# hucancode/hello-raytracing

Hardware: AMD Instinct MI355X
Metric: Mrays/sec at 1920x1080x1024spp x 50-bounce (RTIOW cover scene) (higher is better)
Workload: dtype f32

## Files before the change

hello-raytracing_amd/csrc/rt_kernels.hip:

```cpp
#include "rt_device.hpp"
#include "rt_tile_lists.hpp"

#include <algorithm>
#include <type_traits>

using namespace hrt_dev;

namespace {

struct Ray {
    f3 o, d;
};

#ifdef HRT_STAMPS
__device__ __forceinline__ unsigned long long hrt_stamp() {
    unsigned long long t;
    __builtin_amdgcn_sched_barrier(0);
    asm volatile("s_memtime %0\n\ts_waitcnt lgkmcnt(0)" : "=s"(t)::"memory");
    __builtin_amdgcn_sched_barrier(0);
    return t;
}
__device__ __forceinline__ unsigned long long hrt_realtime() {
    unsigned long long t;
    __builtin_amdgcn_sched_barrier(0);
// ... 237 lines not shown
    const float a4 = 4.0f * a, a2 = 2.0f * a;
    Q.sp = 0;
    const bool finite_o = __builtin_isfinite(r.o.x) && __builtin_isfinite(r.o.y) && __builtin_isfinite(r.o.z);
    if (!(a2 > 0x1p-100f && a2 < 0x1p100f) || !finite_o) {
        Q.full_scan = 1u;
        return false;
    }
    Q.full_scan = 0u;
    const uint32_t nleaf = P.bvh_nleaf;
    float bt = best;
    int bc = -1;
    KPtr K = nullptr;
    if constexpr (LLDS) K = kargs();
    const uint32_t nlarge = LLDS ? K->bq_nlarge : KA ? kargs()->nlarge : P.nlarge;
    if constexpr (LLDS) {
        static_assert(KA && FAST, "k_trace_split's begin");
        for (uint32_t k = 0, n = min(nlarge, LLARGE_CAP); k < n; k++) {
            const float4 g = lgeo[k];
            const bool cand = sphere_candidate(g, r, a4);
            const float t = candidate_t(g, r, a4, a2, cand);
            if (cand && t > 0.0f && t < bt) { bt = t; bc = (int)(nleaf + k); }
        }
    } else
    for (uint32_t k = 0; k < nlarge; k++) {
        const int i = P.large_slots[k];
        float t;
        if constexpr (FAST) {
            const float4 g = P.sph_geo[i];
            const bool cand = sphere_candidate(g, r, a4);
            t = candidate_t(g, r, a4, a2, cand);
            t = cand ? t : -1.0f;
        } else {
            t = exact_t_geo<false>(P.sph_geo[i], r, a4, a2);
        }
        if (beats(t, i, bt, bc >= 0 ? bvh_slot_of(P, bc) : -1)) { bt = t; bc = (int)(nleaf + k); }
    }
    if constexpr (COUNT) tally.spheres += nlarge;
    Q.bt = bt;
    Q.bc = bc;
    if constexpr (LLDS) {
        bvh_slab_k<SO>(r, Q, K->bq_rc, K->bq_rr_h, K->bq_k1, K->bq_k2, K->bq_k3, K->bq_k4);
    } else {
        bvh_slab<SO>(P, r, Q);
    }
    Q.node = P.bvh_root;
    return true;
}

template <bool SO, typename RC>
__device__ __forceinline__ void bvh_slab_k(const Ray& r, BvhQuery& Q, RC rc, float rr, float k1, float k2, float k3, float k4) {
    const float a = dot(r.d, r.d);
    const f3 op = mk(r.o.x - rc[0], r.o.y - rc[1], r.o.z - rc[2]);
    const float dl = __builtin_amdgcn_sqrtf(dot(op, op));
    const float D = dl * 1.001f + rr;
    const float delta = k1 + fmin_ieee(k2 * (D * D), k3 * D) + k4 * D +
                        4.0001e-23f * __builtin_amdgcn_rsqf(a);
    const float pad = 2.02f * delta;
    Q.S.inv = mk(robust_inv(r.d.x), robust_inv(r.d.y), robust_inv(r.d.z));
    if constexpr (SO) {
        const f3 ps = mk(__builtin_copysignf(pad, Q.S.inv.x), __builtin_copysignf(pad, Q.S.inv.y),
                         __builtin_copysignf(pad, Q.S.inv.z));
        Q.S.lo = mk(-op.x - ps.x, -op.y - ps.y, -op.z - ps.z);
        Q.S.hi = mk(-op.x + ps.x, -op.y + ps.y, -op.z + ps.z);
    } else {
        Q.S.lo = mk(-op.x - pad, -op.y - pad, -op.z - pad);
        Q.S.hi = mk(-op.x + pad, -op.y + pad, -op.z + pad);
    }
    Q.S.lo = Q.S.lo * Q.S.inv;
    Q.S.hi = Q.S.hi * Q.S.inv;
}

typedef _Float16 hrt_h2 __attribute__((ext_vector_type(2)));
__device__ __forceinline__ float h16_lo(uint32_t u) { return (float)__builtin_bit_cast(hrt_h2, u).x; }
__device__ __forceinline__ float h16_hi(uint32_t u) { return (float)__builtin_bit_cast(hrt_h2, u).y; }
__device__ __forceinline__ void load_hnode(const uint4* __restrict__ hn, uint32_t node, float4& n0, float4& n1,
                                           float4& n2, float4& n3) {
    const uint4 c0 = hn[2 * node], c1 = hn[2 * node + 1];
    n0 = float4{h16_lo(c0.x), h16_lo(c0.y), h16_lo(c0.z), __uint_as_float(c0.w)};
    n1 = float4{h16_hi(c0.x), h16_hi(c0.y), h16_hi(c0.z), 0.0f};
    n2 = float4{h16_lo(c1.x), h16_lo(c1.y), h16_lo(c1.z), __uint_as_float(c1.w)};
    n3 = float4{h16_hi(c1.x), h16_hi(c1.y), h16_hi(c1.z), 0.0f};
}

__device__ __forceinline__ bool box_hit_so(uint32_t px, uint32_t py, uint32_t pz, uint32_t shx, uint32_t shy, uint32_t shz,
                                           const Slab& S, float bt, float& tenter) {
    const uint32_t x = __builtin_amdgcn_alignbit(px, px, shx), y = __builtin_amdgcn_alignbit(py, py, shy),
                   z = __builtin_amdgcn_alignbit(pz, pz, shz);
    const float tnx = __builtin_fmaf(h16_lo(x), S.inv.x, S.lo.x), tfx = __builtin_fmaf(h16_hi(x), S.inv.x, S.hi.x);
    const float tny = __builtin_fmaf(h16_lo(y), S.inv.y, S.lo.y), tfy = __builtin_fmaf(h16_hi(y), S.inv.y, S.hi.y);
    const float tnz = __builtin_fmaf(h16_lo(z), S.inv.z, S.lo.z), tfz = __builtin_fmaf(h16_hi(z), S.inv.z, S.hi.z);
    const float tmin = fmax_ieee(fmax_ieee(tnx, tny), fmax_ieee(tnz, 0.0f));
    const float tmax = fmin_ieee(fmin_ieee(tfx, tfy), tfz);
    tenter = tmin;
    return tmin <= tmax && tmin <= bt;
}

template <bool FAST>
__device__ __forceinline__ void leaf_sphere_test(const KParams& P, const Ray& r, float a4, float a2, uint32_t i, float& bt,
                                                 int& bc) {
    float4 g;
    if constexpr (FAST) {
        typedef float f4v __attribute__((ext_vector_type(4)));
        const __amdgpu_buffer_rsrc_t rs =
            __builtin_amdgcn_make_buffer_rsrc((void*)P.bvh_sph, (short)0, (int)(P.bvh_nleaf * 16u), 0x00020000);
        const f4v v = __builtin_amdgcn_raw_buffer_load_b128(rs, (int)(i * 16u), 0, 0);
        g = float4{v.x, v.y, v.z, v.w};
    } else {
        g = P.bvh_sph[i];
    }
    const float t = exact_t_geo<FAST>(g, r, a4, a2);
    if (t > 0.0f && t <= bt) {
        int slot;
        if constexpr (FAST) {
            const __amdgpu_buffer_rsrc_t rsl =
                __builtin_amdgcn_make_buffer_rsrc((void*)P.bvh_slot, (short)0, (int)(P.bvh_nleaf * 4u), 0x00020000);
            slot = (int)__builtin_amdgcn_raw_buffer_load_b32(rsl, (int)(i * 4u), 0, 0);
        } else {
            slot = P.bvh_slot[i];
        }
        if (t < bt || (bc >= 0 && slot < bvh_slot_of(P, bc))) { bt = t; bc = (int)i; }
    }
}

template <bool SUSPEND, bool SELECT, uint32_t LS, bool COUNT = true, bool HOLD = false, bool PAIR = false,
          typename SW = uint32_t>
__device__ __forceinline__ bool bvh_walk_noovf(const KParams& P, const Ray& r, BvhQuery& Q, SW* stack, Tally& tally,
                                               uint32_t below, const uint4* __restrict__ hn, uint32_t hold = 0u) {
    constexpr bool S16 = sizeof(SW) == 2;
    const Slab S = Q.S;
    const uint32_t shx = (__float_as_uint(S.inv.x) >> 27) & 16u, shy = (__float_as_uint(S.inv.y) >> 27) & 16u,
                   shz = (__float_as_uint(S.inv.z) >> 27) & 16u;
    const float a = dot(r.d, r.d);
    const float a4 = 4.0f * a, a2 = 2.0f * a;
    uint32_t node = Q.node;
    int sp = Q.sp;
    float bt = Q.bt;
    int bc = Q.bc;
    uint32_t finished = 0u;
#ifdef HRT_STAMPS
    tally.lentry++;
    if (first_active_lane()) tally.wentry++;
#endif
    while (true) {
#ifdef HRT_STAMPS
        tally.lwalk++;
        if (first_active_lane()) tally.wwalk++;
#endif
        uint32_t lim = 0u;
        if constexpr (HOLD) lim = min(hold, (uint32_t)__popcll(__ballot(1)));
        constexpr uint32_t BVH_MISS = 0xFFFFFFFFu;
        if (!(node & BVH_LEAF_BIT)) {
            bool any;
            do {
#ifdef HRT_STAMPS
                {
                    constexpr uint32_t DIAG_LOW = 24u;
                    const bool low = (uint32_t)__popcll(__ballot(1)) < DIAG_LOW;
                    tally.lbox++;
                    tally.lbox_low += low ? 1u : 0u;
                    if (first_active_lane()) {
                        tally.wbox++;
                        tally.wbox_low += low ? 1u : 0u;
                    }
                }
#endif
                float tl, tr;
                const uint4 c0 = hn[2 * node], c1 = hn[2 * node + 1];
                const bool hl = box_hit_so(c0.x, c0.y, c0.z, shx, shy, shz, S, bt, tl);
                const bool hr = box_hit_so(c1.x, c1.y, c1.z, shx, shy, shz, S, bt, tr);
                if constexpr (COUNT) tally.boxes += 2;
                const bool lfirst = hl && (!hr || tl <= tr);
                const uint32_t near = lfirst ? c0.w : c1.w, far = lfirst ? c1.w : c0.w;
                const bool both = hl && hr;
                any = hl || hr;
                stack[sp * LS] = (SW)far;
                sp += both ? 1 : 0;
                node = any ? near : (HOLD ? BVH_MISS : node);
                if constexpr (HOLD) {
                    const unsigned long long wants = __builtin_amdgcn_ballot_w64(!(node & BVH_LEAF_BIT));
                    if (!__builtin_amdgcn_inverse_ballot_w64((uint32_t)__popcll(wants) < lim ? 0ull : wants)) break;
                } else {
                    if (!(any && !(node & BVH_LEAF_BIT))) break;
                }
            } while (true);
        }
        if (HOLD ? (int32_t)node < -1 : (node & BVH_LEAF_BIT) != 0u) {
#ifdef HRT_STAMPS
            {
                constexpr uint32_t DIAG_LOW = 24u;
                const bool low = (uint32_t)__popcll(__ballot(1)) < DIAG_LOW;
                tally.lleaf++;
                tally.lleaf_low += low ? 1u : 0u;
                if (first_active_lane()) {
                    tally.wleaf++;
                    tally.wleaf_low += low ? 1u : 0u;
                }
            }
#endif
            const uint32_t first = (node >> 4) & (S16 ? 0x7FFu : 0x07FFFFFFu), cnt = node & 15u;
            if constexpr (SELECT) {
                typedef float f4v __attribute__((ext_vector_type(4)));
                const __amdgpu_buffer_rsrc_t rs =
                    __builtin_amdgcn_make_buffer_rsrc((void*)P.bvh_sph, (short)0, (int)(P.bvh_nleaf * 16u), 0x00020000);
                auto leaf_geo = [&](uint32_t o) -> float4 {
                    const f4v v = __builtin_amdgcn_raw_buffer_load_b128(rs, (int)o, 0, 0);
                    return float4{v.x, v.y, v.z, v.w};
                };
                uint32_t cand = 0u;
                if constexpr (PAIR) {
                    static_assert(BVH_MAX_LEAF <= 4u, "two pairs cover a leaf");
                    const uint32_t o = first * 16u;
                    HRT_TALLY(lpass1, wpass1);
                    const f4v v0 = __builtin_amdgcn_raw_buffer_load_b128(rs, (int)o, 0, 0);
                    const f4v v1 = __builtin_amdgcn_raw_buffer_load_b128(rs, (int)o, 16, 0);
                    if (sphere_candidate(float4{v0.x, v0.y, v0.z, v0.w}, r, a4)) cand |= 1u;
                    if (sphere_candidate(float4{v1.x, v1.y, v1.z, v1.w}, r, a4)) cand |= 2u;
                    if (cnt > 2u) {
                        HRT_TALLY(lpass1, wpass1);
                        const f4v v2 = __builtin_amdgcn_raw_buffer_load_b128(rs, (int)o, 32, 0);
                        const f4v v3 = __builtin_amdgcn_raw_buffer_load_b128(rs, (int)o, 48, 0);
                        if (sphere_candidate(float4{v2.x, v2.y, v2.z, v2.w}, r, a4)) cand |= 4u;
                        if (sphere_candidate(float4{v3.x, v3.y, v3.z, v3.w}, r, a4)) cand |= 8u;
                    }
                    cand &= ~(~0u << cnt);
                } else {
                    for (uint32_t o = first * 16u, oe = (first + cnt) * 16u, bit = 1u; o != oe; o += 16u, bit <<= 1) {
                        HRT_TALLY(lpass1, wpass1);
                        if (sphere_candidate(leaf_geo(o), r, a4)) cand |= bit;
                    }
                }
#ifdef HRT_STAMPS
                if (cand != 0u) HRT_TALLY(lrun, wrun);
#endif
                while (cand != 0u) {
                    HRT_TALLY(lroot, wroot);
                    const uint32_t o = (first + (uint32_t)__builtin_ctz(cand)) * 16u;
                    cand &= cand - 1u;
                    const float t = candidate_t(leaf_geo(o), r, a4, a2);
                    if (t > 0.0f && t <= bt) {
                        const __amdgpu_buffer_rsrc_t rsl = __builtin_amdgcn_make_buffer_rsrc(
                            (void*)P.bvh_slot, (short)0, (int)(P.bvh_nleaf * 4u), 0x00020000);
                        const int slot = (int)__builtin_amdgcn_raw_buffer_load_b32(rsl, (int)(o >> 2), 0, 0);
                        if (t < bt || (bc >= 0 && slot < bvh_slot_of(P, bc))) { bt = t; bc = (int)(o >> 4); }
                    }
                }
            } else {
                for (uint32_t o = first * 16u, oe = (first + cnt) * 16u; o != oe; o += 16u)
                    leaf_sphere_test<false>(P, r, a4, a2, o >> 4, bt, bc);
            }
            if constexpr (COUNT) tally.spheres += cnt;
        }
        if constexpr (HOLD) {
            const bool held = !(node & BVH_LEAF_BIT);
            const bool fin = !held && sp == 0;
            const int spn = max(sp - 1, 0);
// ... 2093 lines not shown
            } else {
                uint32_t* const rw = rows + 9u * (threadIdx.x >> 6);
                if ((lane & 7u) == 0u) rw[lane >> 3] = (x * K->cam.H + y) * time;
                if (lane == 0u) rw[8] = K->cam.H * time;
            }
            __builtin_amdgcn_fence(__ATOMIC_RELEASE, "wavefront");
            __builtin_amdgcn_wave_barrier();
            __builtin_amdgcn_fence(__ATOMIC_ACQUIRE, "wavefront");
        }
        const uint32_t avail = 64u - B.blk_next;
        const uint32_t rank = (uint32_t)__popcll(m & below);
        const uint32_t src = (B.blk_next + rank) & 63u;
        const float* const e = blk + BW * ((threadIdx.x & ~63u) + src);
        const float ox = e[0], oy = e[1], oz = e[2], dx = e[3], dy = e[4], dz = e[5];
        bool took = false;
        const uint32_t okb = (okw[2u * (threadIdx.x >> 6) + (src >> 5)] >> (src & 31u)) & 1u;
        if (need && rank < avail) {
            need = false;
            if (okb) {
                ray.o = mk(ox, oy, oz);
                ray.d = mk(dx, dy, dz);
                if constexpr (SEED) {
                    s = __float_as_uint(e[6]);
                } else {
                    const uint32_t* const rw = rows + 9u * (threadIdx.x >> 6);
                    uint32_t st = rw[src >> 3] + (src & 7u) * rw[8];
#pragma unroll
                    for (int k = 0; k < 5; k++) st = pcg_next(st);
                    s = st;
                }
                fl = sample_ref<RING>(J, B.job_f0, B.blk_f);
                pix = B.job_tile * 64u + src;
                sky_t = ray.d.y * 0.5f + 0.5f;
                att = mk(1.0f, 1.0f, 1.0f);
                bounce = 0;
                have = true;
                qs = 0;
                took = true;
            }
        }
        job_dealt<RING>(J, (uint32_t)__popcll(__ballot(took)));
        B.blk_next += min((uint32_t)__popcll(m), avail);
        if (B.blk_next == 64u && B.blk_f + 1u >= B.job_nf) job_close(J, lane);
        m = __ballot(need);
    }
}

#ifdef HRT_PHASES
#define HRT_PHASE_DECL                                                                       \
    unsigned long long ph[5] = {0, 0, 0, 0, 0}, pl[4] = {0, 0, 0, 0}, pr[4] = {0, 0, 0, 0}; \
    const unsigned long long ph_start = hrt_stamp();                                         \
    unsigned long long ph_t = ph_start
#define HRT_PHASE(k)                                                                         \
    do {                                                                                     \
        const unsigned long long t_ = hrt_stamp();                                          \
        ph[k] += t_ - ph_t;                                                                  \
        ph_t = t_;                                                                           \
    } while (0)
#define HRT_LANES(k, pred)                                                                   \
    do {                                                                                     \
        const uint32_t c_ = (uint32_t)__popcll(__ballot(pred));                              \
        if (c_) { pl[k] += c_; pr[k]++; }                                                    \
    } while (0)
#define HRT_PHASE_FLUSH                                                                      \
    if (lane == 0) {                                                                         \
        for (int k = 0; k < 4; k++) atomicAdd(P.counter + 8 + k, ph[k]);                     \
        atomicAdd(P.counter + 12, hrt_stamp() - ph_start);                                   \
        for (int k = 0; k < 3; k++) atomicAdd(P.counter + 5 + k, pl[k]);                     \
        atomicAdd(P.counter + 13, pr[0]);                                                    \
        atomicAdd(P.counter + 14, pr[2]);                                                    \
    }
#else
#define HRT_PHASE_DECL do { } while (0)
#define HRT_PHASE(k) do { } while (0)
#define HRT_LANES(k, pred) do { } while (0)
#define HRT_PHASE_FLUSH
#endif

constexpr bool split_stack16(bool lnodes, bool packet) { return lnodes && !packet; }
constexpr int split_waves(bool lnodes, bool steal, bool count, bool packet, bool ring) {
    if (packet) return steal ? 6 : 7;
    return split_stack16(lnodes, packet) && !steal && !count && !ring ? 8 : 7;
}
template <bool LNODES, bool STEAL, bool COUNT, bool PACKET, bool RING>
__device__ __forceinline__ void trace_split(const KParams& P) {
    static_assert(!PACKET || LNODES, "the packet walk reads the LDS nodes and keeps its stack in one VGPR (depth <= 8)");
    constexpr int MODE = MODE_SPHERE;
    constexpr int FM = PACKET ? FOLD_DYN : (int)RING;
    static_assert(!(PACKET && RING) && !(STEAL && RING), "no such instantiation: launch_trace_split");
    constexpr int SPLIT_STACK = LNODES ? (int)LNODE_DEPTH : 14;
    constexpr bool SHADE_BY_CODE = !PACKET;
    constexpr bool SEAMS = !PACKET && !STEAL && !RING;
    constexpr uint32_t QS_IDLE = 0xFFFFFFFFu, QS_PASS = 0xFFFFFFFEu;
    constexpr bool BLOCKRES = SEAMS && !COUNT && LNODES;
    constexpr bool WAVEQ = PACKET || BLOCKRES;
    constexpr uint32_t QS_FULL = 5u;
    const uint32_t lane = threadIdx.x & 63u;
    constexpr bool STACK16 = split_stack16(LNODES, PACKET);
    static_assert(!STACK16 || (LNODE_CAP <= 0x8000u && (LNODE_CAP + 1u) * BVH_MAX_LEAF <= 2048u),
                  "a 16-bit stack entry holds a node index or first << 4 | count in 15 bits");
    using StackWord = std::conditional_t<STACK16, int16_t, uint32_t>;
    __shared__ StackWord bvh_stack[SPLIT_STACK * 256];
    __shared__ uint4 lnodes[LNODES ? 2 * LNODE_CAP : 1];
    constexpr bool LLDS = LNODES && !PACKET;
    __shared__ float4 lgeo[LLDS ? LLARGE_CAP : 1];
    if constexpr (LNODES) {
        const uint32_t nn = 2u * min(P.bvh_nnodes, LNODE_CAP);
        for (uint32_t i = threadIdx.x; i < nn; i += 256u) {
            uint4 c = P.bvh_hnodes[i];
            if constexpr (STACK16) c.w = (uint32_t)(int32_t)(int16_t)(c.w | (c.w >> 16));
            lnodes[i] = c;
        }
        if constexpr (LLDS) {
            if (threadIdx.x < min(P.nlarge, LLARGE_CAP)) {
                lgeo[threadIdx.x] = P.sph_geo[P.large_slots[threadIdx.x]];
            }
        }
        __syncthreads();
    }
    __shared__ float4 blk[2 * 256];
    __shared__ float blk_sky[BLOCKRES ? 256 : 1];
    constexpr uint32_t EW_RES = 0x80000000u;
    Tally tally;
    uint32_t queries = 0;
    const uint32_t suspend_below = P.suspend_below & 0xFFu, hold = P.suspend_below >> 8;

    bool drained = false;
    Ray ray;
    f3 att = mk(1.0f, 1.0f, 1.0f);
    float sky_t = 0.0f;
    uint32_t s = 0, bounce = 0, pix = 0, fl = 0;
    bool have = false;
    uint32_t qs = SEAMS ? QS_IDLE : 0u;
    const auto has = [&]() { return (int)qs >= 0; };
    BvhQuery Q;
    uint32_t job_tile = 0, job_f0 = 0, job_nf = 0, blk_f = 0, blk_next = 64;
    uint32_t blk_cnt = 64;
    uint32_t nres = 0;
    uint32_t nfull = 0;
    const auto blk_n = [&]() { return BLOCKRES ? blk_cnt : 64u; };
    __shared__ uint32_t wjobs[4 * WJ_WORDS];
    const WaveJobs Jp = PACKET ? wave_jobs(wjobs) : WaveJobs{nullptr};
    StackWord* const stack_p = PACKET ? bvh_stack + threadIdx.x : nullptr;
    if (FM != 1 && P.fold_prev != nullptr) fold_prev_tiles(P, lane);
    const WaveJobs J = PACKET ? Jp : wave_jobs(wjobs);
    StackWord* const stack = PACKET ? stack_p : bvh_stack + threadIdx.x;
    const unsigned long long below = (1ull << lane) - 1ull;
    HRT_PHASE_DECL;
#ifdef HRT_STAMPS
    WaveRecord wrec;
    wrec.begin();
    uint32_t nblocks = 0;
#endif
    while (true) {
        if constexpr (SEAMS) qs = (uint32_t)max((int)qs, (int)QS_IDLE);
        bool need = (SEAMS ? qs == QS_IDLE : !have) && !drained;
        unsigned long long m = __ballot(need);
        while (m != 0ull) {
            if (blk_next == blk_n()) {
                if constexpr (STEAL) {
                    if ((uint32_t)__popcll(m) < CLAIM_FREE && J.get(WJ_PRIV_N) == 0u && __ballot(have) != 0ull &&
                        queue_drained(J, lane))
                        break;
                    if (!steal_block(J, lane, job_tile, job_f0)) {
                        drained = steal_drained(J);
                        break;
                    }
                    blk_f = 0;
                    job_nf = 1;
                } else {
                    if (J.dealing()) {
                        blk_f++;
                    } else {
                        if ((J.get(WJ_FLAGS) & WJ_TAILPH) && (uint32_t)__popcll(m) < CLAIM_FREE &&
                            __ballot(SEAMS ? has() : have) != 0ull)
                            break;
                        if (!job_acquire<FM, true>(J, lane, drained, job_tile, job_f0, job_nf)) break;
                        blk_f = 0;
                    }
                }
                blk_next = 0;
#ifdef HRT_STAMPS
                nblocks++;
#endif
                const uint32_t x = (job_tile % P.tiles_w) * 8u + (lane & 7u);
                const uint32_t kr = (job_tile / P.tiles_w) * 8u + (lane >> 3);
                const uint32_t pok = (x < P.W && kr < P.nrows) ? 1u : 0u;
                Ray pr = {mk(0.0f, 0.0f, 0.0f), mk(0.0f, 0.0f, 0.0f)};
                uint32_t ps = 0;
                uint32_t ew = pok;
                if (pok) {
                    const KPtr K = kargs();
                    uint32_t y;
                    if constexpr (SEAMS) {
                        const uint32_t rb = K->row_block, rs = K->row_stride;
                        if (__builtin_expect(rb == rs, 1)) y = K->row0 + kr;
                        else y = global_row(K->row0, rb, rs, kr);
                    } else {
                        y = global_row(K->row0, K->row_block, K->row_stride, kr);
                    }
                    pr = primary_ray<MODE>(&K->cam, x, y, K->time0 + (job_f0 + blk_f) * K->dtime, ps);
                }
                bool resolved = false;
                if constexpr (BLOCKRES) {
                    typedef const __attribute__((address_space(4))) uint32_t* CU32;
                    typedef float f4v __attribute__((ext_vector_type(4)));
                    typedef const __attribute__((address_space(4))) f4v* CF4;
                    blk_cnt = 64u;
                    const KPtr TK = kargs();
                    const CU32 tl = (CU32)TK->tile_lists + uniform(job_tile) * TILE_LIST_WORDS;
                    const uint32_t ln = TK->tile_lists != nullptr ? tl[0] : TILE_LIST_WALK;
                    const float a = dot(pr.d, pr.d);
                    const float a4 = 4.0f * a, a2 = 2.0f * a;
                    const bool cov = (a2 > 0x1p-100f && a2 < 0x1p100f) && __builtin_isfinite(pr.o.x) &&
                                     __builtin_isfinite(pr.o.y) && __builtin_isfinite(pr.o.z);
                    if (ln != TILE_LIST_WALK && __ballot(pok != 0u && !cov) == 0ull) {
                        resolved = true;
                        nres++;
                        blk[2 * threadIdx.x] = float4{ray.o.x, ray.o.y, ray.o.z, ray.d.x};
                        blk[2 * threadIdx.x + 1] = float4{ray.d.y, ray.d.z, __uint_as_float(s), __uint_as_float(pix)};
                        blk_sky[threadIdx.x] = sky_t;
                        const bool live = pok != 0u;
                        float bt = FLT_MAX_REF;
                        int bc = -1;
// ... 120 lines not shown
                            blk[2 * threadIdx.x + 1].w = __uint_as_float(rw);
                        }
                    }
                }
                __builtin_amdgcn_fence(__ATOMIC_RELEASE, "wavefront");
                __builtin_amdgcn_wave_barrier();
                __builtin_amdgcn_fence(__ATOMIC_ACQUIRE, "wavefront");
            }
            const uint32_t avail = blk_n() - blk_next;
            const uint32_t rank = WAVEQ ? __builtin_amdgcn_mbcnt_hi((uint32_t)(m >> 32), __builtin_amdgcn_mbcnt_lo((uint32_t)m, 0u))
                                         : (uint32_t)__popcll(m & below);
            const int src = (int)((blk_next + rank) & 63u);
            const float4 b0 = blk[2 * ((threadIdx.x & ~63u) + (uint32_t)src)];
            const float4 b1 = blk[2 * ((threadIdx.x & ~63u) + (uint32_t)src) + 1];
            const float ox = b0.x, oy = b0.y, oz = b0.z, dx = b0.w, dy = b1.x, dz = b1.y;
            const uint32_t ss = __float_as_uint(b1.z), ok = __float_as_uint(b1.w);
            bool took = false;
            if ((SEAMS ? qs == QS_IDLE : need) && rank < avail) {
                need = false;
                if constexpr (SEAMS) qs = QS_PASS;
                if (ok & 1u) {
                    ray.o = mk(ox, oy, oz);
                    ray.d = mk(dx, dy, dz);
                    s = ss;
                    if constexpr (SEAMS) {
                        pix = (job_f0 + blk_f) * kargs()->sample_npix + job_tile * 64u +
                              (BLOCKRES && (ok & EW_RES) ? (ok >> 1) & 63u : (uint32_t)src);
                    } else {
                        fl = sample_ref<FM>(J, job_f0, blk_f);
                        pix = job_tile * 64u + (uint32_t)src;
                    }
                    sky_t = ray.d.y * 0.5f + 0.5f;
                    att = mk(1.0f, 1.0f, 1.0f);
                    bounce = 0;
                    if constexpr (BLOCKRES) {
                        if (ok & EW_RES) {
                            const SphereAux* const w = P.code_aux + ((ok & ~EW_RES) >> 7);
                            sky_t = blk_sky[(threadIdx.x & ~63u) + (uint32_t)src];
                            att = att * mk(w->ar * 0.7f, w->ag * 0.7f, w->ab * 0.7f);
                            bounce = 1;
                        }
                    }
                    if constexpr (!SEAMS) have = true;
                    qs = 0;
                    if constexpr (PACKET) {
                        if (ok & 2u) {
                            qs = 4u;
                            Q.bc = (ok & 4u) ? (int)(ok >> 3) : -1;
                        }
                    }
                    took = true;
                }
            }
            job_dealt<FM>(J, (uint32_t)__popcll(__ballot(took)));
            blk_next += min((uint32_t)__popcll(m), avail);
            if (blk_next == blk_n() && blk_f + 1u >= job_nf) job_close(J, lane);
            m = __ballot(SEAMS ? qs == QS_IDLE : need);
        }
#ifdef HRT_STAMPS
        wrec.drain(drained);
#endif
        if (__ballot(SEAMS ? has() : have) == 0ull) {
            if (drained && J.idle()) break;
            if (!drained && idle_spin(J, lane)) break;
        }
        bool fin = false;
#ifdef HRT_STAMPS
        if (lane == 0) tally.rounds++;
#endif
        HRT_PHASE(0);
        HRT_LANES(0, (SEAMS ? has() : have) && qs == 0u);
        if (SEAMS ? qs == 0u : have && qs == 0u) {
            if (bounce < P.bounces) {
                qs = bvh_begin<true, true, true, COUNT, LLDS>(P, ray, FLT_MAX_REF, Q, tally, lgeo) ? 1u : BLOCKRES ? QS_FULL : 2u;
            } else {
                qs = 3u;
            }
        }
        HRT_PHASE(1);
        HRT_LANES(1, (SEAMS ? has() : have) && qs == 1u);
        if (SEAMS ? qs == 1u : have && qs == 1u) {
            if constexpr (LNODES) {
                constexpr bool PAIR = !PACKET && !STEAL;
                if (bvh_walk_noovf<true, true, 256, COUNT, !PACKET, PAIR>(P, ray, Q, stack, tally, suspend_below, lnodes, hold))
                    qs = 2u;
            } else {
                if (bvh_walk_ovf<true, SPLIT_STACK, true, 256, true, COUNT>(P, ray, Q, stack, tally, suspend_below, P.bvh_hnodes))
                    qs = 2u;
            }
        }
        HRT_PHASE(2);
        HRT_LANES(2, (SEAMS ? has() : have) && qs >= 2u);
        if constexpr (PACKET) queries += (uint32_t)__popcll(__ballot(have && (qs == 2u || qs == 4u)));
        if constexpr (BLOCKRES) {
            const uint32_t nf = (uint32_t)__popcll(__ballot(qs == QS_FULL));
            queries += (uint32_t)__popcll(__ballot(qs == 2u)) + nf;
            nfull += nf;
        }
        if (SEAMS ? (int)qs >= 2 : have && qs >= 2u) {
#ifdef HRT_STAMPS
            tally.lshade++;
            if (first_active_lane()) tally.wshade++;
#endif
            bool done = true;
            if (qs == 2u || (PACKET && qs == 4u) || (BLOCKRES && qs == QS_FULL)) {
                float best = FLT_MAX_REF;
                int bi;
                f3 p;
                if (PACKET && qs == 4u) {
                    bi = Q.bc;
                    p = ray.o;
                } else if constexpr (SHADE_BY_CODE) {
                    bi = Q.bc;
                    if (BLOCKRES ? qs == QS_FULL : Q.full_scan != 0u) {
                        if constexpr (BLOCKRES) {
                            bi = scan_spheres_p<false>(kargs(), ray, best);
                        } else {
                            bi = bvh_end<true>(P, ray, Q, best, tally);
                        }
                        bi = bi >= 0 ? bi + (int)(P.bvh_nleaf + kargs()->nlarge) : bi;
                    } else {
                        best = Q.bt;
                    }
                    p = point_on_ray(ray.o, ray.d, best);
                } else {
                    bi = bvh_end<true>(P, ray, Q, best, tally);
                    p = point_on_ray(ray.o, ray.d, best);
                }
                if constexpr (!WAVEQ) queries++;
                if (bi >= 0) {
                    Hit h;
                    if constexpr (SEAMS) {
                        const __amdgpu_buffer_rsrc_t rsa =
                            __builtin_amdgcn_make_buffer_rsrc((void*)P.code_aux, (short)0, (int)P.code_aux_bytes, 0x00020000);
                        const int aoff = sphere_record_rs(rsa, p, ray.d, bi, best, h);
                        scatter_dc<MODE, true>(s, ray, h, [&]() {
                            const u32x4 m = __builtin_amdgcn_raw_buffer_load_b128(rsa, aoff, 32, 0);
                            return DielRegs{__uint_as_float(m.y), __uint_as_float(m.z), __uint_as_float(m.w)};
                        });
                    } else {
                        const SphereAux* __restrict__ tab = SHADE_BY_CODE ? P.code_aux : nullptr;
                        sphere_record_p<true>(P, p, ray.d, bi, best, h, tab);
                        scatter<MODE, true>(P, s, ray, h, tab);
                    }
                    att = att * mk(h.ar * 0.7f, h.ag * 0.7f, h.ab * 0.7f);
                    bounce++;
                    done = bounce >= P.bounces;
                }
            }
            if (done) {
                const float u = 1.0f - sky_t;
                const f3 sky = mk(0.54f * u + 0.54f * sky_t, 0.86f * u + 0.7f * sky_t, 0.92f * u + 0.98f * sky_t);
                const f3 c = att * sky;
                if constexpr (SEAMS) {
                    const KPtr RK = kargs();
                    float* const o = RK->samples + (unsigned long long)pix * 3u;
#if defined(HRT_STAMPS) && defined(HRT_DIAG_NOSTORE)
                    if (c.x == -12345.0f)
#endif
                    {
                        o[0] = c.x;
                        o[1] = c.y;
                        o[2] = c.z;
                    }
                    if (uint32_t* const tc = RK->tile_cost)
                        __hip_atomic_fetch_add(tc + pix % RK->sample_npix, bounce + 1u, __ATOMIC_RELAXED, __HIP_MEMORY_SCOPE_AGENT);
                } else {
                    ring_store<FM>(J, pix, fl, c, bounce + 1u);
                }
                if constexpr (!SEAMS) have = false;
                fin = true;
            }
            qs = SEAMS && done ? QS_IDLE : 0u;
        }
        job_account<FM, 1>(J, fin, fl, lane);
        HRT_PHASE(3);
    }
#ifdef HRT_STAMPS
    wrec.finish(P, lane, nblocks);
#endif
    HRT_PHASE_FLUSH
#if defined(HRT_STAMPS) && !defined(HRT_PHASES)
    {
#ifdef HRT_LEAFSTAT
        unsigned long long v[10] = {tally.lbox, tally.wbox, tally.lleaf, tally.wleaf, tally.lpass1, tally.wpass1,
                                    tally.lrun, tally.wrun, tally.lroot, tally.wroot};
#else
        unsigned long long v[10] = {tally.lbox, tally.wbox, tally.lleaf, tally.wleaf, tally.rounds, tally.lshade,
                                    tally.wshade, tally.lwalk, tally.wwalk, tally.lentry};
#endif
#pragma unroll
        for (int c = 0; c < 10; c++) {
#pragma unroll
            for (int off = 32; off > 0; off >>= 1) v[c] += __shfl_xor(v[c], off);
        }
        if (lane == 0)
            for (int c = 0; c < 10; c++) atomicAdd(P.counter + 5 + c, v[c]);
    }
#endif
#ifdef HRT_RINGSTAT
    if (lane == 0)
        for (uint32_t c = 0; c < 4u; c++) atomicAdd(P.counter + 5 + c, (unsigned long long)J.get(WJ_STAT + c));
#endif
    if constexpr (BLOCKRES) {
        if (lane == 0) {
            unsigned long long sums[6] = {queries, 0ull, (unsigned long long)nfull * kargs()->nslots, 0ull, 0ull, nres};
            flush_counts(sums);
        }
        return;
    }
    unsigned long long sums[5] = {(!WAVEQ || lane == 0u) ? queries : 0u, tally.boxes, tally.spheres, tally.nodes, tally.tris};
#pragma unroll
    for (int c = 0; c < 5; c++) {
#pragma unroll
        for (int off = 32; off > 0; off >>= 1) sums[c] += __shfl_xor(sums[c], off);
    }
    if (lane == 0) flush_counts(sums);
}
template <bool LNODES, bool STEAL, bool COUNT, bool PACKET>
__global__ __launch_bounds__(256) __attribute__((amdgpu_waves_per_eu(split_waves(LNODES, STEAL, COUNT, PACKET, false)))) void
k_trace_split(const KParams P) {
    trace_split<LNODES, STEAL, COUNT, PACKET, false>(P);
}
template <bool LNODES, bool COUNT>
__global__ __launch_bounds__(256) __attribute__((amdgpu_waves_per_eu(split_waves(LNODES, false, COUNT, false, true)))) void
k_ring_split(const KParams P) {
    trace_split<LNODES, false, COUNT, false, true>(P);
}

constexpr uint32_t heap_wg(int hl) { return hl == 3 ? 768u : 256u; }
constexpr uint32_t heap_list_words(int hl, int scan) { return hl == 0 ? TRI_BATCH : (hl == 3 && scan != SCAN_BVH) ? 7u : 8u; }
constexpr uint32_t heap_top_n(int hl, int scan) { return hl == 0 ? 0u : hl == 1 ? 256u : 1024u; }

template <int MODE, int SCAN, int HL, bool STEAL, bool RING>
__device__ __forceinline__ void trace_split_tris(const KParams& P) {
    static_assert(MODE != MODE_SPHERE, "k_trace_split covers the sphere program");
    constexpr uint32_t WGT = heap_wg(HL), HT = heap_top_n(HL, SCAN);
    const uint32_t lane = threadIdx.x & 63u;
    constexpr uint32_t LIST_WORDS = heap_list_words(HL, SCAN);
    constexpr int SPHERE_STACK = (int)LIST_WORDS;
    static_assert(SCAN != SCAN_BVH || HL == 0 || LIST_WORDS == 8, "the culling walk's stack needs 8 entries");
    __shared__ uint32_t lane_words[LIST_WORDS * WGT];
    uint32_t* const cand = lane_words + threadIdx.x;
    uint32_t* const sstack = lane_words + threadIdx.x;
    __shared__ float heap_top[HL > 0 ? 9 * HT : 1];
    if constexpr (HL > 0) {
        const uint32_t nf = 9u * min(P.n, HT);
        for (uint32_t t = threadIdx.x; t < nf; t += WGT) heap_top[t] = P.nodes_so[t];
        __syncthreads();
    }
    uint16_t* defer_list = nullptr;
    if constexpr (SCAN == SCAN_DEFER) {
        static_assert(HL <= 1, "the deferred scan's lists assume 256-lane workgroups");
        __shared__ uint16_t defer_cand[(CAND_CAP + 1) * 256];
        defer_list = defer_cand + threadIdx.x;
    }
    Tally tally;
    uint32_t queries = 0;
    const unsigned long long below = (1ull << lane) - 1ull;
    const uint32_t suspend_below = P.suspend_below;

    constexpr bool SEED = !(HL == 3 && SCAN == SCAN_BVH);
    __shared__ float blk[(SEED ? 7 : 6) * WGT];
    __shared__ uint32_t blk_rows[SEED ? 1 : 9 * (WGT / 64u)];
    __shared__ uint32_t blk_ok[2 * (WGT / 64u)];
    BlockState B;
    __shared__ uint32_t wjobs[(WGT / 64u) * WJ_WORDS];
    const WaveJobs J = wave_jobs(wjobs);
    if (P.fold_prev != nullptr) fold_prev_tiles(P, lane);
    bool drained = false;
    Ray ray;
    f3 att = mk(1.0f, 1.0f, 1.0f);
    float sky_t = 0.0f;
    uint32_t s = 0, bounce = 0, pix = 0, fl = 0;
    bool have = false;
    uint32_t qs = 0;
    HeapWalk W;
    HRT_PHASE_DECL;
#ifdef HRT_STAMPS
    WaveRecord wrec;
    wrec.begin();
#endif
    while (true) {
        refill_block_lds<MODE, STEAL, SEED, RING>(P, B, J, blk, blk_rows, blk_ok, drained, lane, below, have, qs, ray, att, sky_t, s,
                                            bounce, pix, fl);
#ifdef HRT_STAMPS
        wrec.drain(drained);
#endif
        if (__ballot(have) == 0ull) {
            if (drained && J.idle()) break;
            if (!drained && idle_spin(J, lane)) break;
        }
        HRT_PHASE(0);
        HRT_LANES(0, have && qs == 0u);
        bool fin = false;
        if (have && qs == 0u) {
            if (bounce >= P.bounces) {
                qs = 5u;
            } else if constexpr (MODE == MODE_TRIS) {
                heap_begin(ray, FLT_MAX_REF, W);
                qs = 3u;
            } else {
                float sb = FLT_MAX_REF;
// ... 625 lines not shown
    static int cus = 0;
    if (cus == 0) {
        int dev = 0;
        hipError_t e = hipGetDevice(&dev);
        if (e == hipSuccess) e = hipDeviceGetAttribute(&cus, hipDeviceAttributeMultiprocessorCount, dev);
        if (e != hipSuccess) return e;
    }
    int per_cu = 0;
    hipError_t e = hipOccupancyMaxActiveBlocksPerMultiprocessor(&per_cu, kernel, (int)wgt, 0);
    if (e != hipSuccess) return e;
    const unsigned long long wpb = wgt / 64u;
    const unsigned long long want = (P.njobs + wpb - 1ull) / wpb;
    const unsigned long long cap = (unsigned long long)std::max(1, per_cu) * (unsigned long long)cus;
    const dim3 grid((unsigned)std::min(want, std::min(cap, (unsigned long long)P.steal_cap / wpb)));
    KParams Q = P;
    Q.nwaves = (uint32_t)(grid.x * wpb);
    hipLaunchKernelGGL(kernel, grid, dim3((unsigned)wgt), 0, stream, Q);
    return hipGetLastError();
}

template <int MODE, int SCAN, int HL>
static hipError_t launch_split_tris_hl(const KParams& P, hipStream_t stream) {
    const char* base = "k_trace_split_tris";
    if (P.steal) return launch_persistent(k_trace_split_tris<MODE, SCAN, HL, true>, P, stream, kname_iiib(base, MODE, SCAN, HL, 1), heap_wg(HL));
    return P.ring_mode ? launch_persistent(k_ring_split_tris<MODE, SCAN, HL>, P, stream, kname_iiib(base, MODE, SCAN, HL, 0), heap_wg(HL))
                       : launch_persistent(k_trace_split_tris<MODE, SCAN, HL, false>, P, stream, kname_iiib(base, MODE, SCAN, HL, 0), heap_wg(HL));
}
template <int MODE, int SCAN>
static hipError_t launch_split_tris(const KParams& P, hipStream_t stream) {
    if constexpr (SCAN == SCAN_DEFER) {
        if (P.tri_small > 1u) return hipErrorInvalidValue;
        return P.tri_small ? launch_split_tris_hl<MODE, SCAN, 1>(P, stream) : launch_split_tris_hl<MODE, SCAN, 0>(P, stream);
    } else {
        if (P.tri_small != 0u && P.tri_small != 3u) return hipErrorInvalidValue;
        return P.tri_small ? launch_split_tris_hl<MODE, SCAN, 3>(P, stream) : launch_split_tris_hl<MODE, SCAN, 0>(P, stream);
    }
}

template <int MODE, int SCAN, bool TSAH>
struct KernelSel {
    static constexpr int mode = MODE, scan = SCAN;
    static constexpr bool tsah = TSAH;
};
template <int MODE, bool TSAH, typename F>
static auto with_scan(int variant, F&& f) {
    if constexpr (MODE == MODE_TRIS) {
        return f(KernelSel<MODE, SCAN_SIMPLE, TSAH>{});
    } else {
        if (variant == SCAN_SIMPLE) return f(KernelSel<MODE, SCAN_SIMPLE, TSAH>{});
        if (variant == SCAN_DEFER) return f(KernelSel<MODE, SCAN_DEFER, TSAH>{});
        return f(KernelSel<MODE, SCAN_BVH, TSAH>{});
    }
}
template <typename F>
static auto with_scene_kernel(int mode, int variant, bool tri_bvh, F&& f) {
    switch (mode) {
    case MODE_SPHERE: return with_scan<MODE_SPHERE, false>(variant, f);
    case MODE_TRIS: return tri_bvh ? with_scan<MODE_TRIS, true>(variant, f) : with_scan<MODE_TRIS, false>(variant, f);
    default: return tri_bvh ? with_scan<MODE_MIXED, true>(variant, f) : with_scan<MODE_MIXED, false>(variant, f);
    }
}

template <int MODE, int SCAN, bool TSAH>
static hipError_t launch_k_trace(const KParams& P, hipStream_t stream) {
    const char* name = kname("k_trace", MODE, SCAN, (int)TSAH);
    return P.ring_mode ? launch_persistent(k_ring<MODE, SCAN, TSAH>, P, stream, name)
                       : launch_persistent(k_trace<MODE, SCAN, TSAH>, P, stream, name);
}

template <bool COUNT>
static hipError_t launch_trace_split(const KParams& P, hipStream_t stream) {
    const char* base = "k_trace_split";
    if (P.ring_mode && !(P.bvh_lnodes && P.packet)) {
        return P.bvh_lnodes ? launch_persistent(k_ring_split<true, COUNT>, P, stream, kname_bbbb(base, 1, 0, COUNT, 0))
                            : launch_persistent(k_ring_split<false, COUNT>, P, stream, kname_bbbb(base, 0, 0, COUNT, 0));
    }
    if (P.bvh_lnodes && P.packet) {
        return P.steal ? launch_persistent(k_trace_split<true, true, COUNT, true>, P, stream, kname_bbbb(base, 1, 1, COUNT, 1))
                       : launch_persistent(k_trace_split<true, false, COUNT, true>, P, stream, kname_bbbb(base, 1, 0, COUNT, 1));
    }
    if (P.steal)
        return P.bvh_lnodes ? launch_persistent(k_trace_split<true, true, COUNT, false>, P, stream, kname_bbbb(base, 1, 1, COUNT, 0))
                            : launch_persistent(k_trace_split<false, true, COUNT, false>, P, stream, kname_bbbb(base, 0, 1, COUNT, 0));
    return P.bvh_lnodes ? launch_persistent(k_trace_split<true, false, COUNT, false>, P, stream, kname_bbbb(base, 1, 0, COUNT, 0))
                        : launch_persistent(k_trace_split<false, false, COUNT, false>, P, stream, kname_bbbb(base, 0, 0, COUNT, 0));
}

hipError_t hrt_launch_trace(int mode, int variant, const KParams& P, hipStream_t stream) {
    if (P.njobs == 0) return hipSuccess;
    const bool split_kernel = mode == MODE_SPHERE ? (variant == SCAN_BVH && P.suspend_below > 0u) : !P.tri_bvh;
    if (P.tail_from != 0xFFFFFFFFu && !(split_kernel && !P.steal && !P.ring_mode)) return hipErrorInvalidValue;
    if (P.steal && P.ring_mode) return hipErrorInvalidValue;
    if (mode == MODE_SPHERE && variant == SCAN_BVH && P.suspend_below > 0u)
        return P.count_tests ? launch_trace_split<true>(P, stream) : launch_trace_split<false>(P, stream);
    return with_scene_kernel(mode, variant, P.tri_bvh != 0, [&](auto sel) -> hipError_t {
        if constexpr (sel.mode != MODE_SPHERE && !sel.tsah) {
            if (P.suspend_below == 0u) return hipErrorInvalidValue;
            return launch_split_tris<sel.mode, sel.scan>(P, stream);
        } else if constexpr (sel.mode == MODE_SPHERE && sel.scan == SCAN_BVH) {
            return hipErrorInvalidValue;
        } else {
            return launch_k_trace<sel.mode, sel.scan, sel.tsah>(P, stream);
        }
    });
}

hipError_t hrt_launch_render(int mode, int variant, const KParams& P, hipStream_t stream) {
    const dim3 grid((P.W + 15u) / 16u, (P.nrows + 15u) / 16u);
    if (grid.x == 0 || grid.y == 0) return hipSuccess;
    with_scene_kernel(mode, variant, P.tri_bvh != 0, [&](auto sel) {
        (void)kname("k_render", sel.mode, sel.mode == MODE_TRIS ? SCAN_SIMPLE : variant, (int)sel.tsah);
        hipLaunchKernelGGL((k_render<sel.mode, sel.scan, sel.tsah>), grid, dim3(256), 0, stream, P);
    });
    return hipGetLastError();
}

static dim3 ray_grid(uint32_t n) { return dim3((uint32_t)(((unsigned long long)n + 255u) / 256u)); }

hipError_t hrt_launch_cast(int mode, int variant, const KParams& P, const float* origins, const float* dirs, uint32_t n,
                           void* hits, hipStream_t stream) {
    if (n == 0) return hipSuccess;
    with_scene_kernel(mode, variant, P.tri_bvh != 0, [&](auto sel) {
        hipLaunchKernelGGL((k_cast_rays<sel.mode, sel.scan, sel.tsah>), ray_grid(n), dim3(256), 0, stream, P, origins, dirs, n,
                           (uint4*)hits);
    });
    return hipGetLastError();
}

hipError_t hrt_launch_bounce(int mode, int variant, const KParams& P, const BounceIO& io, uint32_t n, hipStream_t stream) {
    if (n == 0) return hipSuccess;
    with_scene_kernel(mode, variant, P.tri_bvh != 0, [&](auto sel) {
        hipLaunchKernelGGL((k_bounce_rays<sel.mode, sel.scan, sel.tsah>), ray_grid(n), dim3(256), 0, stream, P, io, n);
    });
    return hipGetLastError();
}

hipError_t hrt_launch_occluded(int mode, int variant, const KParams& P, const float* origins, const float* dirs,
                               const float* tmax, uint32_t n, void* occluded, hipStream_t stream) {
    if (n == 0) return hipSuccess;
    with_scene_kernel(mode, variant, P.tri_bvh != 0, [&](auto sel) {
        hipLaunchKernelGGL((k_occluded<sel.mode, sel.scan, sel.tsah>), ray_grid(n), dim3(256), 0, stream, P, origins, dirs, tmax, n,
                           (uint8_t*)occluded);
    });
    return hipGetLastError();
}

hipError_t hrt_launch_trace_rays(int mode, int variant, const KParams& P, const float* origins, const float* dirs,
                                 const uint32_t* rng, uint32_t seed, uint32_t n, uint32_t R, float* radiance, uint32_t* queries,
                                 hipStream_t stream) {
    if (n == 0) return hipSuccess;
    if (R == 0) R = 1;
    const unsigned long long waves = ((unsigned long long)n + 64ull * R - 1u) / (64ull * R);
    const dim3 grid((uint32_t)((waves + 3u) / 4u));
    with_scene_kernel(mode, variant, P.tri_bvh != 0, [&](auto sel) {
        hipLaunchKernelGGL((k_radiance_rays<sel.mode, sel.scan, sel.tsah>), grid, dim3(256), 0, stream, P, origins, dirs, rng, seed,
                           n, R, radiance, queries);
    });
    return hipGetLastError();
}

hipError_t hrt_launch_primary_rays(int mode, const KParams& P, uint32_t time, float* origins, float* dirs, uint32_t* state,
                                   hipStream_t stream) {
    const unsigned long long n = (unsigned long long)P.nrows * P.W;
    if (n == 0) return hipSuccess;
    dim3 block(256);
    dim3 grid((uint32_t)((n + 255u) / 256u));
    switch (mode) {
// ... 13 lines not shown
```

Measured before the change: 56660.

## Pre-rotate LDS BVH nodes per ray direction sign and use 512-lane workgroups

The BLOCKRES split kernel stores each BVH node in LDS in a 64-byte pre-rotated layout that keeps both the plain and the half-swapped halves of each axis. Each ray then folds its direction-sign offsets into per-axis LDS base addresses, so a box test does one 16-byte and two 8-byte LDS reads and skips the per-child alignbit rotations. The same kernel variant moves from 256 to 512-thread workgroups so more waves share each LDS node copy. The cost is twice the LDS per node, which lowers the node cap or occupancy, plus an assumption that the launch helper accepts the new workgroup size argument.

```diff
diff --git a/hello-raytracing_amd/csrc/rt_kernels.hip b/hello-raytracing_amd/csrc/rt_kernels.hip
--- a/hello-raytracing_amd/csrc/rt_kernels.hip
+++ b/hello-raytracing_amd/csrc/rt_kernels.hip
@@ -343,10 +343,7 @@
     n3 = float4{h16_hi(c1.x), h16_hi(c1.y), h16_hi(c1.z), 0.0f};
 }
 
-__device__ __forceinline__ bool box_hit_so(uint32_t px, uint32_t py, uint32_t pz, uint32_t shx, uint32_t shy, uint32_t shz,
-                                           const Slab& S, float bt, float& tenter) {
-    const uint32_t x = __builtin_amdgcn_alignbit(px, px, shx), y = __builtin_amdgcn_alignbit(py, py, shy),
-                   z = __builtin_amdgcn_alignbit(pz, pz, shz);
+__device__ __forceinline__ bool box_hit_near(uint32_t x, uint32_t y, uint32_t z, const Slab& S, float bt, float& tenter) {
     const float tnx = __builtin_fmaf(h16_lo(x), S.inv.x, S.lo.x), tfx = __builtin_fmaf(h16_hi(x), S.inv.x, S.hi.x);
     const float tny = __builtin_fmaf(h16_lo(y), S.inv.y, S.lo.y), tfy = __builtin_fmaf(h16_hi(y), S.inv.y, S.hi.y);
     const float tnz = __builtin_fmaf(h16_lo(z), S.inv.z, S.lo.z), tfz = __builtin_fmaf(h16_hi(z), S.inv.z, S.hi.z);
@@ -354,6 +351,21 @@
     const float tmax = fmin_ieee(fmin_ieee(tfx, tfy), tfz);
     tenter = tmin;
     return tmin <= tmax && tmin <= bt;
+}
+__device__ __forceinline__ bool box_hit_so(uint32_t px, uint32_t py, uint32_t pz, uint32_t shx, uint32_t shy, uint32_t shz,
+                                           const Slab& S, float bt, float& tenter) {
+    const uint32_t x = __builtin_amdgcn_alignbit(px, px, shx), y = __builtin_amdgcn_alignbit(py, py, shy),
+                   z = __builtin_amdgcn_alignbit(pz, pz, shz);
+    return box_hit_near(x, y, z, S, bt, tenter);
+}
+
+constexpr uint32_t PREROT_NODE_BYTES = 64u;
+__device__ __forceinline__ void prerot_node(uint4* dst, const uint4 c0, const uint4 c1) {
+    const auto rot = [](uint32_t p) { return __builtin_amdgcn_alignbit(p, p, 16u); };
+    dst[0] = uint4{c0.x, c1.x, c0.w, c1.w};
+    dst[1] = uint4{rot(c0.x), rot(c1.x), c0.w, c1.w};
+    dst[2] = uint4{c0.y, c1.y, rot(c0.y), rot(c1.y)};
+    dst[3] = uint4{c0.z, c1.z, rot(c0.z), rot(c1.z)};
 }
 
 template <bool FAST>
@@ -384,13 +396,23 @@
 }
 
 template <bool SUSPEND, bool SELECT, uint32_t LS, bool COUNT = true, bool HOLD = false, bool PAIR = false,
-          typename SW = uint32_t>
+          typename SW = uint32_t, bool PREROT = false>
 __device__ __forceinline__ bool bvh_walk_noovf(const KParams& P, const Ray& r, BvhQuery& Q, SW* stack, Tally& tally,
                                                uint32_t below, const uint4* __restrict__ hn, uint32_t hold = 0u) {
     constexpr bool S16 = sizeof(SW) == 2;
     const Slab S = Q.S;
-    const uint32_t shx = (__float_as_uint(S.inv.x) >> 27) & 16u, shy = (__float_as_uint(S.inv.y) >> 27) & 16u,
-                   shz = (__float_as_uint(S.inv.z) >> 27) & 16u;
+    typedef uint32_t w4v __attribute__((ext_vector_type(4)));
+    typedef uint32_t w2v __attribute__((ext_vector_type(2)));
+    typedef const __attribute__((address_space(3))) w4v* LdsU4;
+    typedef const __attribute__((address_space(3))) w2v* LdsU2;
+    uint32_t shx = (__float_as_uint(S.inv.x) >> 27) & 16u, shy = (__float_as_uint(S.inv.y) >> 27) & 16u,
+             shz = (__float_as_uint(S.inv.z) >> 27) & 16u;
+    if constexpr (PREROT) {
+        const uint32_t hb = (uint32_t)(uintptr_t)(const __attribute__((address_space(3))) void*)hn;
+        shx = hb + shx;
+        shy = hb + 32u + (shy >> 1);
+        shz = hb + 48u + (shz >> 1);
+    }
     const float a = dot(r.d, r.d);
     const float a4 = 4.0f * a, a2 = 2.0f * a;
     uint32_t node = Q.node;
@@ -426,12 +448,30 @@
                 }
 #endif
                 float tl, tr;
-                const uint4 c0 = hn[2 * node], c1 = hn[2 * node + 1];
-                const bool hl = box_hit_so(c0.x, c0.y, c0.z, shx, shy, shz, S, bt, tl);
-                const bool hr = box_hit_so(c1.x, c1.y, c1.z, shx, shy, shz, S, bt, tr);
+                bool hl, hr;
+                uint32_t w0, w1;
+                if constexpr (PREROT) {
+                    static_assert(PREROT_NODE_BYTES == 64u, "the shift below");
+                    uint32_t ax, ay, az;
+                    asm("v_lshl_add_u32 %0, %1, 6, %2" : "=v"(ax) : "v"(node), "v"(shx));
+                    asm("v_lshl_add_u32 %0, %1, 6, %2" : "=v"(ay) : "v"(node), "v"(shy));
+                    asm("v_lshl_add_u32 %0, %1, 6, %2" : "=v"(az) : "v"(node), "v"(shz));
+                    const w4v gx = *(LdsU4)(uintptr_t)ax;
+                    const w2v gy = *(LdsU2)(uintptr_t)ay, gz = *(LdsU2)(uintptr_t)az;
+                    hl = box_hit_near(gx.x, gy.x, gz.x, S, bt, tl);
+                    hr = box_hit_near(gx.y, gy.y, gz.y, S, bt, tr);
+                    w0 = gx.z;
+                    w1 = gx.w;
+                } else {
+                    const uint4 c0 = hn[2 * node], c1 = hn[2 * node + 1];
+                    hl = box_hit_so(c0.x, c0.y, c0.z, shx, shy, shz, S, bt, tl);
+                    hr = box_hit_so(c1.x, c1.y, c1.z, shx, shy, shz, S, bt, tr);
+                    w0 = c0.w;
+                    w1 = c1.w;
+                }
                 if constexpr (COUNT) tally.boxes += 2;
                 const bool lfirst = hl && (!hr || tl <= tr);
-                const uint32_t near = lfirst ? c0.w : c1.w, far = lfirst ? c1.w : c0.w;
+                const uint32_t near = lfirst ? w0 : w1, far = lfirst ? w1 : w0;
                 const bool both = hl && hr;
                 any = hl || hr;
                 stack[sp * LS] = (SW)far;
@@ -2691,6 +2731,12 @@
     if (packet) return steal ? 6 : 7;
     return split_stack16(lnodes, packet) && !steal && !count && !ring ? 8 : 7;
 }
+constexpr bool split_prerot(bool lnodes, bool steal, bool count, bool packet, bool ring) {
+    return lnodes && !steal && !count && !packet && !ring;
+}
+constexpr uint32_t split_wg(bool lnodes, bool steal, bool count, bool packet, bool ring) {
+    return split_prerot(lnodes, steal, count, packet, ring) ? 512u : 256u;
+}
 template <bool LNODES, bool STEAL, bool COUNT, bool PACKET, bool RING>
 __device__ __forceinline__ void trace_split(const KParams& P) {
     static_assert(!PACKET || LNODES, "the packet walk reads the LDS nodes and keeps its stack in one VGPR (depth <= 8)");
@@ -2709,13 +2755,25 @@
     static_assert(!STACK16 || (LNODE_CAP <= 0x8000u && (LNODE_CAP + 1u) * BVH_MAX_LEAF <= 2048u),
                   "a 16-bit stack entry holds a node index or first << 4 | count in 15 bits");
     using StackWord = std::conditional_t<STACK16, int16_t, uint32_t>;
-    __shared__ StackWord bvh_stack[SPLIT_STACK * 256];
-    __shared__ uint4 lnodes[LNODES ? 2 * LNODE_CAP : 1];
+    constexpr bool PREROT = split_prerot(LNODES, STEAL, COUNT, PACKET, RING);
+    constexpr uint32_t WG = split_wg(LNODES, STEAL, COUNT, PACKET, RING);
+    static_assert(PREROT == BLOCKRES, "the 512-lane workgroup and the pre-rotated nodes: the BLOCKRES kernel's");
+    __shared__ StackWord bvh_stack[SPLIT_STACK * WG];
+    __shared__ uint4 lnodes[LNODES ? (PREROT ? PREROT_NODE_BYTES / 16u : 2u) * LNODE_CAP : 1];
     constexpr bool LLDS = LNODES && !PACKET;
     __shared__ float4 lgeo[LLDS ? LLARGE_CAP : 1];
     if constexpr (LNODES) {
         const uint32_t nn = 2u * min(P.bvh_nnodes, LNODE_CAP);
-        for (uint32_t i = threadIdx.x; i < nn; i += 256u) {
+        if constexpr (PREROT) {
+            static_assert(STACK16, "the child words sign-extended, as below");
+            for (uint32_t i = threadIdx.x; 2u * i < nn; i += WG) {
+                uint4 c0 = P.bvh_hnodes[2u * i], c1 = P.bvh_hnodes[2u * i + 1u];
+                c0.w = (uint32_t)(int32_t)(int16_t)(c0.w | (c0.w >> 16));
+                c1.w = (uint32_t)(int32_t)(int16_t)(c1.w | (c1.w >> 16));
+                prerot_node(lnodes + (PREROT_NODE_BYTES / 16u) * i, c0, c1);
+            }
+        } else
+        for (uint32_t i = threadIdx.x; i < nn; i += WG) {
             uint4 c = P.bvh_hnodes[i];
             if constexpr (STACK16) c.w = (uint32_t)(int32_t)(int16_t)(c.w | (c.w >> 16));
             lnodes[i] = c;
@@ -2727,8 +2785,8 @@
         }
         __syncthreads();
     }
-    __shared__ float4 blk[2 * 256];
-    __shared__ float blk_sky[BLOCKRES ? 256 : 1];
+    __shared__ float4 blk[2 * WG];
+    __shared__ float blk_sky[BLOCKRES ? WG : 1];
     constexpr uint32_t EW_RES = 0x80000000u;
     Tally tally;
     uint32_t queries = 0;
@@ -2748,7 +2806,7 @@
     uint32_t nres = 0;
     uint32_t nfull = 0;
     const auto blk_n = [&]() { return BLOCKRES ? blk_cnt : 64u; };
-    __shared__ uint32_t wjobs[4 * WJ_WORDS];
+    __shared__ uint32_t wjobs[(WG / 64u) * WJ_WORDS];
     const WaveJobs Jp = PACKET ? wave_jobs(wjobs) : WaveJobs{nullptr};
     StackWord* const stack_p = PACKET ? bvh_stack + threadIdx.x : nullptr;
     if (FM != 1 && P.fold_prev != nullptr) fold_prev_tiles(P, lane);
@@ -3035,10 +3093,11 @@
         if (SEAMS ? qs == 1u : have && qs == 1u) {
             if constexpr (LNODES) {
                 constexpr bool PAIR = !PACKET && !STEAL;
-                if (bvh_walk_noovf<true, true, 256, COUNT, !PACKET, PAIR>(P, ray, Q, stack, tally, suspend_below, lnodes, hold))
+                if (bvh_walk_noovf<true, true, WG, COUNT, !PACKET, PAIR, StackWord, PREROT>(P, ray, Q, stack, tally, suspend_below,
+                                                                                            lnodes, hold))
                     qs = 2u;
             } else {
-                if (bvh_walk_ovf<true, SPLIT_STACK, true, 256, true, COUNT>(P, ray, Q, stack, tally, suspend_below, P.bvh_hnodes))
+                if (bvh_walk_ovf<true, SPLIT_STACK, true, WG, true, COUNT>(P, ray, Q, stack, tally, suspend_below, P.bvh_hnodes))
                     qs = 2u;
             }
         }
@@ -3171,7 +3230,8 @@
     if (lane == 0) flush_counts(sums);
 }
 template <bool LNODES, bool STEAL, bool COUNT, bool PACKET>
-__global__ __launch_bounds__(256) __attribute__((amdgpu_waves_per_eu(split_waves(LNODES, STEAL, COUNT, PACKET, false)))) void
+__global__ __launch_bounds__(split_wg(LNODES, STEAL, COUNT, PACKET, false))
+__attribute__((amdgpu_waves_per_eu(split_waves(LNODES, STEAL, COUNT, PACKET, false)))) void
 k_trace_split(const KParams P) {
     trace_split<LNODES, STEAL, COUNT, PACKET, false>(P);
 }
@@ -3963,7 +4023,8 @@
     if (P.steal)
         return P.bvh_lnodes ? launch_persistent(k_trace_split<true, true, COUNT, false>, P, stream, kname_bbbb(base, 1, 1, COUNT, 0))
                             : launch_persistent(k_trace_split<false, true, COUNT, false>, P, stream, kname_bbbb(base, 0, 1, COUNT, 0));
-    return P.bvh_lnodes ? launch_persistent(k_trace_split<true, false, COUNT, false>, P, stream, kname_bbbb(base, 1, 0, COUNT, 0))
+    return P.bvh_lnodes ? launch_persistent(k_trace_split<true, false, COUNT, false>, P, stream, kname_bbbb(base, 1, 0, COUNT, 0),
+                                            split_wg(true, false, COUNT, false, false))
                         : launch_persistent(k_trace_split<false, false, COUNT, false>, P, stream, kname_bbbb(base, 0, 0, COUNT, 0));
 }
 
```

After: 58190, median of 6. 1.03x the previous value.
